# polli-labs/linnaeus

Hardware: AMD Instinct MI355X
Metric: images/sec (train fwd+bwd) mFormerV1_sm 3x224x224 (higher is better)
Workload: dtype bf16; 1 GPU; mFormerV1_sm train step (forward + 4-task CE loss + backward + AdamW (one HIP launch)), bf16 operands / fp32 accumulate+residual, batch 256/GPU, 3x224x224 synthetic, DropPath 0.2, gradient checkpointing off; per_gpu_batch=256, global_batch=256, parallelism=dp1, grad_mode=direct

## Files before the change

### include/lnx.h

```cpp
#ifndef LNX_H
#define LNX_H
#include <stdint.h>

#ifdef __cplusplus
extern "C" {
#endif

#define LNX_F32 0
#define LNX_BF16 1

const char* lnx_last_error(void);
int lnx_version(void);
int lnx_device_cus(void);
int lnx_set_cu_margin(int cus);
int lnx_set_deterministic(int on);
int lnx_get_deterministic(void);
int lnx_tile_sched_static(void);

typedef struct lnx_rowmap {
    int group, pad, off;
} lnx_rowmap;

enum { LNX_ACT_NONE = 0, LNX_ACT_GELU = 1, LNX_ACT_RELU = 2, LNX_ACT_GELU_BWD = 3, LNX_ACT_RELU_BWD = 4,
       LNX_ACT_GELU_D = 5, LNX_ACT_MUL_AUX = 6 };
// ... 898 lines not shown
    const float* mean;
    const float* rstd;
    float* d_ln_w;
    float* d_ln_b;
    float* ws;
    int64_t ws_floats;
    int dz_plain;
    int ln_defer;
    const int* perm;
    const int* m_dev;
} lnx_convmlp_bwd_args;
int lnx_convmlp_bwd(const lnx_convmlp_bwd_args* args, void* stream);
int64_t lnx_convmlp_bwd_ws_floats(int C, int M);


#define LNX_MAX_META 8
#define LNX_MAX_TASKS 16
typedef struct lnx_mformer_cfg {
    int dtype;
    int batch, img_h, img_w, in_chans;
    int dims[4];
    int conv_depths[2];
    int rope_depths[2];
    int rope_heads[2];
    int mlp_hidden[2];
    int n_meta;
    int meta_dims[LNX_MAX_META];
    int only_last_cls;
    int n_tasks;
    int task_classes[LNX_MAX_TASKS];
// ... 54 lines not shown
```

### linnaeus_amd/_lib.py

```python
from __future__ import annotations

import ctypes as C
import os

_HERE = os.path.dirname(os.path.abspath(__file__))
LIB_PATH = os.environ.get("LNX_LIB_PATH") or os.path.join(_HERE, "liblnx_hip.so")

F32, BF16 = 0, 1
ACT_NONE, ACT_GELU, ACT_RELU, ACT_GELU_BWD, ACT_RELU_BWD, ACT_GELU_D, ACT_MUL_AUX = 0, 1, 2, 3, 4, 5, 6
TN_WS_FLOATS = 256 * (256 * 128 + 256)
DROP_PARTITION_MAX = 64


def drop_list_ints(B: int) -> int:
    return 2 * B + 2
ADDR_PLAIN, ADDR_PATCH2 = 0, 1


class LnxError(RuntimeError):
    pass


class RowMap(C.Structure):
    _fields_ = [("group", C.c_int), ("pad", C.c_int), ("off", C.c_int)]
# ... 357 lines not shown
            _lib.lnx_plan_unit_name.argtypes = [C.c_void_p, C.c_int]
            _lib.lnx_plan_unit_name.restype = C.c_char_p
            _lib.lnx_plan_set_trainable.argtypes = [C.c_void_p, C.c_char_p]
        if hasattr(_lib, "lnx_plan_set_input_grads"):
            _lib.lnx_plan_set_input_grads.argtypes = [C.c_void_p, C.c_int, C.c_int]
            _lib.lnx_plan_input_grads.argtypes = [C.c_void_p]
            _lib.lnx_plan_bind_input_grads.argtypes = [C.c_void_p, C.c_void_p, C.c_void_p]
            _lib.lnx_stem_dgrad.argtypes = [C.POINTER(StemDgradArgs), C.c_void_p]
            _lib.lnx_col2im_stem.argtypes = [C.c_void_p, C.c_int, C.c_int, C.c_int, C.c_int, C.c_int, C.c_int, C.c_void_p, C.c_void_p]
            _lib.lnx_meta_input_grad.argtypes = [C.POINTER(MetaInputGradArgs), C.c_int, C.c_void_p, C.c_int, C.c_int, C.c_void_p]
        if hasattr(_lib, "lnx_gemm_tn_query"):
            _lib.lnx_gemm_tn_query.argtypes = [C.POINTER(WgradArgs), C.POINTER(TnLaunch)]
        if hasattr(_lib, "lnx_layernorm_fwd_query"):
            _lib.lnx_layernorm_fwd_query.argtypes = [C.POINTER(LnArgs), C.POINTER(LnLaunch)]
            _lib.lnx_layernorm_bwd_query.argtypes = [C.POINTER(LnBwdArgs), C.POINTER(LnLaunch)]
        older = bool(os.environ.get("LNX_LIB_PATH")) and os.environ.get("LNX_LIB_OLDER") == "1"
        for name in EXPORTS:
            if not hasattr(_lib, name) and not older:
                raise LnxError(f"{LIB_PATH} does not export {name}; rebuild it")
    return _lib


def set_deterministic(on: bool) -> bool:
    return bool(lib().lnx_set_deterministic(1 if on else 0))


def is_deterministic() -> bool:
    return bool(lib().lnx_get_deterministic())


# ... 11 lines not shown
ATTN_KERNEL_NONE, ATTN_KERNEL_RES4, ATTN_KERNEL_RES8, ATTN_KERNEL_TILED4, ATTN_KERNEL_TILED8 = range(5)

EXPORTS = [
    "lnx_last_error", "lnx_version", "lnx_device_cus", "lnx_set_cu_margin", "lnx_set_deterministic", "lnx_get_deterministic", "lnx_tile_sched_static",
    "lnx_gemm_nt", "lnx_last_nt_kernel", "lnx_nt_kernel_launches", "lnx_nt_dispatch", "lnx_gemm_tn", "lnx_gemm_tn_query", "lnx_gemm_tn_flush", "lnx_gemm_tn_discard", "lnx_amax", "lnx_quantize_fp8", "lnx_gemm_nt_fp8", "lnx_quantize_mxfp8", "lnx_gemm_nt_mxfp8", "lnx_dropout_mul", "lnx_dropout_residual", "lnx_plan_dropout_bytes", "lnx_plan_set_dropout", "lnx_plan_attn_dropout_bytes", "lnx_plan_set_attn_dropout",
    "lnx_layernorm_fwd", "lnx_layernorm_bwd", "lnx_layernorm_bwd_flush", "lnx_layernorm_bwd_discard", "lnx_layernorm_fwd_query", "lnx_layernorm_bwd_query",
    "lnx_dwconv7_fwd", "lnx_dwconv7_fwd_kept", "lnx_dwconv7_wgrad", "lnx_dwconv7_wgrad_kept", "lnx_dwconv7_wgrad_ws_floats",
    "lnx_gemm_nt_group_ok", "lnx_gemm_nt_group", "lnx_rope_cos_table", "lnx_rope_cos_table_hd", "lnx_rope_cossin_table_hd", "lnx_rope_cos_tables", "lnx_attn_bwd_ws_floats", "lnx_attn_bwd_ws_floats_hd", "lnx_attn_fwd", "lnx_attn_bwd", "lnx_attn_bwd_sized", "lnx_attn_fwd_compact", "lnx_attn_bwd_compact", "lnx_attn_bwd_flush", "lnx_attn_bwd_discard", "lnx_attn_dispatch", "lnx_last_attn_kernel", "lnx_last_attn_bwd_launches",
    "lnx_im2col_stem", "lnx_scale_cast", "lnx_scale_cast_compact", "lnx_drop_partition", "lnx_copy_dropped_rows", "lnx_set_drop_compact", "lnx_drop_compact_branches", "lnx_drop_compact_conv_blocks", "lnx_set_last_cls", "lnx_last_cls_blocks", "lnx_layerscale_bwd", "lnx_layerscale_bwd_ws", "lnx_layerscale_bwd_ws_floats", "lnx_layerscale_apply_wgrad", "lnx_fill_rows", "lnx_colsum_rows",
    "lnx_agg2_fwd", "lnx_agg2_bwd", "lnx_pack_meta", "lnx_meta_heads_supported", "lnx_meta_heads_fwd", "lnx_meta_heads_bwd", "lnx_meta_heads_bwd_part_floats", "lnx_prep_weights", "lnx_prep_blocks", "lnx_softce", "lnx_softce_multi", "lnx_taxonomy_rows", "lnx_stem_fwd", "lnx_stem_fwd_ok", "lnx_adamw_blocks", "lnx_grad_sumsq", "lnx_adamw_step", "lnx_ademamix_step", "lnx_sgd_step", "lnx_optim_launches", "lnx_grad_sumsq_guarded", "lnx_adamw_step_guarded", "lnx_ademamix_step_guarded", "lnx_sgd_step_guarded", "lnx_muon_layout", "lnx_muon_step", "lnx_muon_launches", "lnx_muon_partition", "lnx_muon_orthogonalize", "lnx_muon_apply_packed", "lnx_gradnorm_sumsq", "lnx_gradnorm_update",
    "lnx_metrics_table_sizes", "lnx_metrics_update", "lnx_predict", "lnx_resize_taps", "lnx_resize_coeffs", "lnx_preprocess_scratch_bytes", "lnx_preprocess", "lnx_hier_loss_fwd", "lnx_hier_loss_bwd",
    "lnx_hier_refine_fwd", "lnx_hier_refine_bwd", "lnx_hier_refine_launches",
    "lnx_abstain_act", "lnx_ppo_advantages", "lnx_ppo_loss_fwd", "lnx_ppo_loss_bwd", "lnx_abstain_launches",
    "lnx_mix_rows", "lnx_mix_meta", "lnx_meta_mask",
    "lnx_aug_pointwise", "lnx_aug_saturation", "lnx_aug_rowstat", "lnx_aug_rescale", "lnx_aug_affine", "lnx_aug_stencil", "lnx_erase_rects", "lnx_u8hwc_to_f32chw",
    "lnx_convmlp_supported", "lnx_convmlp_fwd", "lnx_convmlp_bwd", "lnx_convmlp_bwd_ws_floats",
    "lnx_plan_create", "lnx_plan_destroy", "lnx_plan_workspace_bytes", "lnx_plan_num_params", "lnx_plan_param_name",
    "lnx_plan_param_numel", "lnx_plan_num_drop_calls", "lnx_plan_logits_numel", "lnx_plan_logits_offset", "lnx_plan_logits_ld",
    "lnx_plan_bind", "lnx_plan_forward", "lnx_plan_forward_tail", "lnx_plan_trunk_valid", "lnx_plan_backward", "lnx_plan_backward_into", "lnx_plan_segment_params", "lnx_plan_profile_begin", "lnx_plan_profile_end", "lnx_plan_profile_begin_spans", "lnx_plan_profile_end_ex", "lnx_plan_set_wgrad_stream", "lnx_plan_set_meta_stream",
    "lnx_plan_num_units", "lnx_plan_unit_name", "lnx_plan_param_unit", "lnx_plan_set_trainable", "lnx_plan_first_trained_unit", "lnx_plan_last_backward_units",
    "lnx_stem_dgrad_ok", "lnx_stem_dgrad", "lnx_col2im_stem", "lnx_meta_input_grad", "lnx_plan_set_input_grads", "lnx_plan_input_grads", "lnx_plan_bind_input_grads",
]


class MetaHeadArgs(C.Structure):
    _fields_ = [
        ("B", C.c_int), ("C", C.c_int), ("dim", C.c_int), ("off", C.c_int),
        ("meta", C.c_void_p), ("meta_width", C.c_int), ("eps", C.c_float),
        ("w0", C.c_void_p), ("ldw0", C.c_int), ("b0", C.c_void_p), ("ln0_w", C.c_void_p), ("ln0_b", C.c_void_p),
        ("w1", C.c_void_p), ("ldw1", C.c_int), ("b1", C.c_void_p), ("ln1_w", C.c_void_p), ("ln1_b", C.c_void_p),
        ("w2", C.c_void_p), ("ldw2", C.c_int), ("b2", C.c_void_p), ("ln2_w", C.c_void_p), ("ln2_b", C.c_void_p),
# ... 124 lines not shown


class ConvMlpBwdArgs(C.Structure):
    _fields_ = [
        ("dtype", C.c_int), ("M", C.c_int), ("C", C.c_int),
        ("g", C.c_void_p), ("ln", C.c_void_p), ("z", C.c_void_p), ("w1", C.c_void_p), ("b1", C.c_void_p),
        ("w2t", C.c_void_p), ("w1t", C.c_void_p), ("gamma", C.c_void_p), ("rowscale", C.c_void_p), ("rows_per_sample", C.c_int),
        ("act", C.c_void_p), ("dh", C.c_void_p), ("dz", C.c_void_p), ("dln", C.c_void_p), ("dgamma", C.c_void_p),
        ("y", C.c_void_p), ("ln_w", C.c_void_p), ("mean", C.c_void_p), ("rstd", C.c_void_p), ("d_ln_w", C.c_void_p), ("d_ln_b", C.c_void_p),
        ("ws", C.c_void_p), ("ws_floats", C.c_int64),
        ("dz_plain", C.c_int), ("ln_defer", C.c_int),
        ("perm", C.c_void_p), ("m_dev", C.c_void_p),
    ]


class StemArgs(C.Structure):
    _fields_ = [("x", C.c_void_p), ("w", C.c_void_p), ("bias", C.c_void_p), ("ln_w", C.c_void_p), ("ln_b", C.c_void_p), ("patches", C.c_void_p),
                ("pre", C.c_void_p), ("y", C.c_void_p), ("mean", C.c_void_p), ("rstd", C.c_void_p), ("B", C.c_int), ("Cin", C.c_int), ("H", C.c_int),
                ("W", C.c_int), ("Cout", C.c_int), ("eps", C.c_float)]


class StemDgradArgs(C.Structure):
    _fields_ = [("dtype", C.c_int), ("B", C.c_int), ("Cin", C.c_int), ("H", C.c_int), ("W", C.c_int), ("Cout", C.c_int),
                ("dy", C.c_void_p), ("ldy", C.c_int64), ("w", C.c_void_p), ("dx", C.c_void_p)]


class MetaInputGradArgs(C.Structure):
    _fields_ = [("B", C.c_int), ("C", C.c_int), ("dim", C.c_int), ("off", C.c_int), ("dp0", C.c_void_p), ("lddp0", C.c_int64), ("w0", C.c_void_p), ("ldw0", C.c_int)]


# ... 20 lines not shown
```

### linnaeus_amd/csrc/api.cpp

```cpp
#include <hip/hip_runtime.h>
#include <stdarg.h>
#include <stdio.h>
#include <stdlib.h>
#include <string.h>

#include <atomic>
#include <mutex>

#include "../../include/lnx.h"

static thread_local char g_err[1024] = "";

void lnx_set_error(const char* fmt, ...) {
    va_list ap;
    va_start(ap, fmt);
    vsnprintf(g_err, sizeof(g_err), fmt, ap);
    va_end(ap);
}

extern "C" const char* lnx_last_error(void) { return g_err; }
extern "C" int lnx_version(void) { return 121; }
extern "C" int lnx_device_cus(void) {
    int dev = 0;
    if (hipGetDevice(&dev) != hipSuccess) return -1;
    hipDeviceProp_t prop;
    if (hipGetDeviceProperties(&prop, dev) != hipSuccess) return -1;
    return prop.multiProcessorCount;
}

static std::atomic<int> g_cu_margin{-1};
int persistent_cus(int cus) {
    int m = g_cu_margin.load(std::memory_order_relaxed);
    if (m < 0) {
        const char* e = getenv("LNX_CU_MARGIN");
        m = e ? atoi(e) : 0;
        if (m < 0) m = 0;
// ... 60 lines not shown
```

### linnaeus_amd/csrc/common.hpp

```cpp
#pragma once
#include <hip/hip_runtime.h>
#include <stdint.h>
#include <stdio.h>

typedef __bf16 bf16_t;
typedef __attribute__((ext_vector_type(8))) __bf16 bf16x8_t;
typedef __attribute__((ext_vector_type(4))) float f32x4_t;

#define LNX_WAVE 64

void lnx_set_error(const char* fmt, ...);

#define LNX_CHECK(cond, ...)                 \
    do {                                     \
        if (!(cond)) {                       \
            lnx_set_error(__VA_ARGS__);      \
            return 1;                        \
        }                                    \
    } while (0)

#define LNX_HIP(expr)                                                                  \
    do {                                                                               \
        hipError_t e_ = (expr);                                                        \
        if (e_ != hipSuccess) {                                                        \
// ... 220 lines not shown
#pragma unroll
    for (int i = 0; i < N; ++i) {
        const f32x2_t u = v[i] * splat2(K);
        const f32x2_t nuu = -(u * u);
        ex[i].x = __builtin_amdgcn_exp2f(nuu.x);
        ex[i].y = __builtin_amdgcn_exp2f(nuu.y);
    }
    erf_sqrt2_poly2_n<N>(v, e);
#pragma unroll
    for (int i = 0; i < N; ++i) {
        const f32x2_t cdf = e[i] * splat2(0.5f) + splat2(0.5f);
        act[i] = v[i] * cdf;
        dgelu[i] = (v[i] * splat2(0.39894228040143267794f)) * ex[i] + cdf;
    }
}
template <int K>
__device__ __forceinline__ void gelu4_bias_n(f32x4_t* h, const f32x4_t* b) {
    f32x2_t v[2 * K], a[2 * K];
#pragma unroll
    for (int k = 0; k < K; ++k) {
        v[2 * k] = f32x2_t{h[k][0] + b[k][0], h[k][1] + b[k][1]};
        v[2 * k + 1] = f32x2_t{h[k][2] + b[k][2], h[k][3] + b[k][3]};
    }
    gelu_lean2_n<2 * K>(v, a);
#pragma unroll
    for (int k = 0; k < K; ++k) h[k] = f32x4_t{a[2 * k].x, a[2 * k].y, a[2 * k + 1].x, a[2 * k + 1].y};
}
template <int K>
__device__ __forceinline__ void gelu4_bias_grad_n(f32x4_t* h, const f32x4_t* b, f32x4_t* da) {
    f32x2_t v[2 * K], a[2 * K], d[2 * K];
// ... 117 lines not shown
```

### linnaeus_amd/csrc/convmlp.hip

```cpp
#include <stdlib.h>

#include "common.hpp"
#include "../../include/lnx.h"

namespace {

struct CmP {
    const unsigned char* ln;
    const unsigned char* w1;
    const unsigned char* w2;
    const unsigned char* w2t;
    const unsigned char* w1t;
    const unsigned char* zin;
    const float* b1;
    const float* b2;
    const float* gamma;
    const float* rowscale;
    const float* x;
    const float* g;
    float* out;
    unsigned char* z;
    unsigned char* act;
    unsigned char* dh;
    unsigned char* dz;
// ... 941 lines not shown
                const float z0 = o[ct][mt][0] + b2.x, z1 = o[ct][mt][1] + b2.y, z2 = o[ct][mt][2] + b2.z, z3 = o[ct][mt][3] + b2.w;
                if constexpr (SAVE == 1) {
                    uint2 zz;
                    bf16_t* zh = reinterpret_cast<bf16_t*>(&zz);
                    zh[0] = (bf16_t)z0; zh[1] = (bf16_t)z1; zh[2] = (bf16_t)z2; zh[3] = (bf16_t)z3;
                    *reinterpret_cast<uint2*>(p.z + ((int64_t)m * C + c) * 2) = zz;
                }
                *reinterpret_cast<float4*>(p.out + (int64_t)m * C + c) =
                    make_float4(xr.x + rs * gm.x * z0, xr.y + rs * gm.y * z1, xr.z + rs * gm.z * z2, xr.w + rs * gm.w * z3);
            }
        }
    }
    if (reset_ctr && lane == 0) sched_reset(ctr);
}

template <int NK, int MT, bool ST, bool LNB, bool DG>
__global__ __launch_bounds__(512) void convmlp_bwd_res_kernel(const CmP p) {
    constexpr int C = Geo<NK>::C;
    constexpr int CT = Geo<NK>::CT;
    constexpr int PART = Geo<NK>::PART;
    constexpr int NCH = 4 * C / 64;
    extern __shared__ __attribute__((aligned(16))) unsigned char smem[];
    unsigned char* w1img = smem;
    unsigned char* w2timg = smem + NCH * PART;
    float* b1s = reinterpret_cast<float*>(smem + 2 * NCH * PART);
    float* dgs = b1s + 4 * C;
    float* lws = dgs + C;
    float* dls = lws + C;
    float* gms = dls + 2 * C;
    const int lane = threadIdx.x & 63;
    const int wave = __builtin_amdgcn_readfirstlane(threadIdx.x >> 6);
// ... 122 lines not shown
                for (int n2 = 0; n2 < 4; n2 += 2) {
                    f32x4_t hv[2] = {h[n2][mt], h[n2 + 1][mt]}, dv[2] = {da[n2][mt], da[n2 + 1][mt]};
                    gelu4_bias_grad_n<2>(hv, &bv[n2], dv);
                    h[n2][mt] = hv[0];
                    h[n2 + 1][mt] = hv[1];
                    da[n2][mt] = dv[0];
                    da[n2 + 1][mt] = dv[1];
                }
            uint4 pd[MT][2];
#pragma unroll
            for (int mt = 0; mt < MT; ++mt) {
                const uint4 pa0 = pack8(h[0][mt], h[1][mt]), pa1 = pack8(h[2][mt], h[3][mt]);
                pd[mt][0] = pack8(da[0][mt], da[1][mt]);
                pd[mt][1] = pack8(da[2][mt], da[3][mt]);
                const int m = min(m_base + mt * 16 + s, Me - 1);
                if constexpr (ST) {
                    const int64_t off = ((int64_t)m * (4 * C) + 64 * j + 8 * g) * 2;
                    st16(p.act + off, pa0);
                    st16(p.act + off + 64, pa1);
                    st16(p.dh + off, pd[mt][0]);
                    st16(p.dh + off + 64, pd[mt][1]);
                }
            }
            prod_tr_nmajor<NK, MT>(dl, lds0 + j * PART, s, g, pd);
        }
        __builtin_amdgcn_sched_barrier(0);
        if (dyn) {
            next = __builtin_amdgcn_readfirstlane(drawn);
            reset_ctr = reset_ctr || next == last_draw;
        } else {
            next = pos + xwaves;
        }
        fetch_tile(cur, next < xcnt ? xbase + next : tile);
        if constexpr (LNB) {
// ... 116 lines not shown
    if (p.y) return p.z ? launch_fwd_res_t<NK, true, 1>(p, st) : (p.ln_out ? launch_fwd_res_t<NK, true, 2>(p, st) : launch_fwd_res_t<NK, true, 0>(p, st));
    return p.z ? launch_fwd_res_t<NK, false, 1>(p, st) : launch_fwd_res_t<NK, false, 0>(p, st);
}
inline int reduce_ln_partials(const CmP& p, int nwg, hipStream_t st) {
    if (deterministic()) {
        ln_fold_rows(p.part, nwg, p.C, p.dlnw, p.dlnb, st);
        return 0;
    }
    if (p.ln_defer) {
        ln_postpone_reduce(p.part, nwg, p.C, p.dlnw, p.dlnb, nwg >= 64 ? 64 : 1, st);
        return 0;
    }
    hipLaunchKernelGGL(ln_partials_reduce_kernel, dim3(cdiv(2 * p.C, 256), nwg >= 64 ? 64 : 1), dim3(256), 0, st, p.part, nwg, p.C, p.dlnw, p.dlnb);
    return 0;
}
template <int NK, int MT, bool ST, bool LNB, bool DG>
int launch_bwd_res_t(const CmP& p, hipStream_t st) {
    const size_t lds0 = 2 * (4 * Geo<NK>::C / 64) * Geo<NK>::PART + 9 * Geo<NK>::C * sizeof(float);
    const size_t lds_det = lds0 + (LNB ? 8 * 2 * Geo<NK>::C * sizeof(float) : 0);
    static bool attr = false;
    if (!attr) {
        (void)hipFuncSetAttribute(reinterpret_cast<const void*>(&convmlp_bwd_res_kernel<NK, MT, ST, LNB, DG>), hipFuncAttributeMaxDynamicSharedMemorySize, (int)lds_det);
        attr = true;
    }
    int grid = bwd_grid(p.C, p.M);
    CmP q = p;
    if (bwd_scratch<LNB, DG>(q, grid) != 0) return -1;
    const int room = res_room();
    if (grid > room) grid = room;
    q.tile_slot = tile_sched_static() ? -1 : tile_slot_of(st);
    hipLaunchKernelGGL((convmlp_bwd_res_kernel<NK, MT, ST, LNB, DG>), dim3(grid), dim3(512), q.det ? lds_det : lds0, st, q);
    fold_dgamma(q, grid, st);
    return LNB ? reduce_ln_partials(p, q.det ? grid * 8 : grid, st) : 0;
}
template <int NK, int MT>
int launch_bwd_res(const CmP& p, hipStream_t st) {
    if (p.zin == nullptr) {
        if (p.y) return p.act ? launch_bwd_res_t<NK, MT, true, true, false>(p, st) : launch_bwd_res_t<NK, MT, false, true, false>(p, st);
        return p.act ? launch_bwd_res_t<NK, MT, true, false, false>(p, st) : launch_bwd_res_t<NK, MT, false, false, false>(p, st);
    }
    if (p.y) return p.act ? launch_bwd_res_t<NK, MT, true, true, true>(p, st) : launch_bwd_res_t<NK, MT, false, true, true>(p, st);
    return p.act ? launch_bwd_res_t<NK, MT, true, false, true>(p, st) : launch_bwd_res_t<NK, MT, false, false, true>(p, st);
}

template <int NK, int MT, int NW, bool LNF>
int launch_fwd_t(const CmP& p, hipStream_t st) {
    const size_t lds = 3 * 2 * Geo<NK>::PART + 4 * Geo<NK>::C * sizeof(float);
    static bool attr = false;
    if (!attr) {
        (void)hipFuncSetAttribute(reinterpret_cast<const void*>(&convmlp_fwd_kernel<NK, MT, NW, LNF>), hipFuncAttributeMaxDynamicSharedMemorySize, (int)lds);
        attr = true;
    }
    hipLaunchKernelGGL((convmlp_fwd_kernel<NK, MT, NW, LNF>), dim3(cdiv(p.M, 16 * NW * MT)), dim3(64 * NW), lds, st, p);
    return 0;
}
template <int NK, int MT, int NW>
int launch_fwd(const CmP& p, hipStream_t st) {
// ... 57 lines not shown
    hipStream_t st = (hipStream_t)stream;
    switch (a->C) {
        case 32: launch_fwd_res<1>(p, st); break;
        case 64: launch_fwd_res<2>(p, st); break;
        case 96: launch_fwd_res<3>(p, st); break;
        case 128: if (nw8) launch_fwd<4, 1, 8>(p, st); else launch_fwd<4, 1, 4>(p, st); break;
        case 192: if (nw8) launch_fwd<6, 1, 8>(p, st); else launch_fwd<6, 1, 4>(p, st); break;
    }
    LNX_LAUNCH_CHECK();
    return 0;
}

extern "C" int lnx_convmlp_bwd(const lnx_convmlp_bwd_args* a, void* stream) {
    LNX_CHECK(a && a->g && a->ln && a->w1 && a->w2t && a->w1t && a->b1 && a->gamma && a->dz && a->dln && (a->dgamma || !a->z),
              "lnx_convmlp_bwd: null operand (z may be NULL: dgamma is then not produced here; with z, dgamma is required)");
    LNX_CHECK((a->act == nullptr) == (a->dh == nullptr), "lnx_convmlp_bwd: act and dh must both be given or both be NULL");
    LNX_CHECK(lnx_convmlp_supported(a->dtype, a->C), "lnx_convmlp_bwd: unsupported dtype %d / C %d", a->dtype, a->C);
    LNX_CHECK(a->M > 0, "lnx_convmlp_bwd: empty");
    if (a->rowscale) LNX_CHECK(a->rows_per_sample > 0, "lnx_convmlp_bwd: rowscale needs rows_per_sample");
    if (a->z && deterministic()) LNX_CHECK(a->ws, "lnx_convmlp_bwd: deterministic mode needs ws (lnx_convmlp_bwd_ws_floats) for the waves' dgamma partial sums");
    if (a->y) LNX_CHECK(a->ln_w && a->mean && a->rstd && a->d_ln_w && a->d_ln_b && a->ws, "lnx_convmlp_bwd: the fused LayerNorm form needs ln_w, mean, rstd, d_ln_w, d_ln_b and ws");
    CmP p{};
    p.y = (const unsigned char*)a->y; p.lnw = a->ln_w; p.mean = const_cast<float*>(a->mean); p.rstd = const_cast<float*>(a->rstd);
    p.part = a->ws; p.part_floats = a->ws_floats; p.dlnw = a->d_ln_w; p.dlnb = a->d_ln_b; p.ln_defer = a->ln_defer;
    p.g = a->g; p.ln = (const unsigned char*)a->ln; p.zin = (const unsigned char*)a->z; p.w1 = (const unsigned char*)a->w1;
    p.w2t = (const unsigned char*)a->w2t; p.w1t = (const unsigned char*)a->w1t; p.b1 = a->b1; p.gamma = a->gamma; p.rowscale = a->rowscale;
    p.act = (unsigned char*)a->act; p.dh = (unsigned char*)a->dh; p.dz = (unsigned char*)a->dz; p.dln = (unsigned char*)a->dln; p.dgamma = a->dgamma;
    p.M = a->M; p.C = a->C; p.rps = a->rows_per_sample > 0 ? a->rows_per_sample : 1;
    p.dz_plain = a->dz_plain != 0;
    LNX_CHECK((a->perm == nullptr) == (a->m_dev == nullptr), "lnx_convmlp_bwd: perm and m_dev go together");
    if (a->perm) LNX_CHECK(a->rows_per_sample > 0 && a->M % a->rows_per_sample == 0 && a->z == nullptr, "lnx_convmlp_bwd: compact rows need rows_per_sample | M and no z");
    p.perm = a->perm; p.m_dev = a->m_dev;
// ... 14 lines not shown
```

### linnaeus_amd/csrc/plan.cpp

```cpp
#include <hip/hip_runtime.h>
#include <stdlib.h>
#include <string.h>

#include <mutex>
#include <atomic>
#include <string>
#include <vector>

#include "../../include/lnx.h"

void lnx_set_error(const char* fmt, ...);

#define RUN(expr)                  \
    do {                           \
        const int rc_ = (expr);    \
        if (rc_ != 0) return rc_;  \
    } while (0)
#define FAIL(...)                   \
    do {                            \
        lnx_set_error(__VA_ARGS__); \
        return 1;                   \
    } while (0)
#define HIPRUN(expr)                                                         \
    do {                                                                     \
// ... 1888 lines not shown
    const int M = B * H * W;
    void* sA = c.at<void>(p->o_sA);
    void* sC = c.at<void>(p->o_sC);
    void* sD = c.at<void>(p->o_sD);
    Timed span(c, 9, 4.0 * M * C * (8.0 * C + 49.0));
    bool forked = false, joined = false;
    const Compact cl = conv_compact_of(p, s, i);
    if (k.fused) {
        void* sB = c.at<void>(p->o_sB);
        lnx_convmlp_bwd_args f;
        memset(&f, 0, sizeof f);
        f.dtype = c.dt; f.M = M; f.C = C;
        f.g = g; f.ln = c.at<void>(k.ln); f.w1 = c.wptr(k.w1); f.b1 = p->P[k.b1];
        f.w2t = c.wtptr(k.w2); f.w1t = c.wtptr(k.w1); f.gamma = p->P[k.gamma];
        f.rowscale = p->drop_ptr(p->drop_conv[s][i]); f.rows_per_sample = H * W;
        f.act = sB; f.dh = sA; f.dz = sC; f.dln = sD; f.dgamma = p->G[k.gamma];
        f.dz_plain = 1;
        f.perm = cl.perm; f.m_dev = cl.m_dev;
        if (k.fused_ln) {
            f.y = c.at<void>(k.y); f.ln_w = p->P[k.lnw]; f.mean = c.at<float>(k.mean); f.rstd = c.at<float>(k.rstd);
            f.d_ln_w = p->G[k.lnw]; f.d_ln_b = p->G[k.lnb];
            f.ws = c.at<float>(p->o_lnws); f.ws_floats = p->lnws_floats;
            if (p->ln_defer && p->o_lnws_defer != 0 && lnx_convmlp_bwd_ws_floats(C, M) <= p->lnws_defer_floats) {
                RUN(ln_defer_slot(c, f.ws, f.ws_floats));
                f.ln_defer = 1;
            }
        }
        {
            Timed t(c, 7, 2.0 * M * C * 4 * C * 3);
            RUN(lnx_convmlp_bwd(&f, c.st));
        }
        const Ctx cw = wg_ctx(c);
        RUN(wg_fork(c, 0));
        forked = true;
        float* S = c.at<float>(p->o_lsws);
        float* T = S + (int64_t)C * 4 * C;
        HIPRUN(hipMemsetAsync(S, 0, ((size_t)C * 4 * C + C) * 4, (hipStream_t)cw.st));
        RUN(wgrad_into(cw, M, C, 4 * C, sC, C, sB, 4 * C, S, T, 4 * C, 0, cl.m_dev));
        RUN(wgrad(cw, M, 4 * C, C, sA, 4 * C, c.at<void>(k.ln), C, k.w1.param, k.b1, C, 0, 1, cl.m_dev));
        RUN(lnx_gemm_tn_flush(cw.st));
        RUN(lnx_layerscale_apply_wgrad(S, T, 4 * C, p->P[k.w2.param], p->P[k.b2], 4 * C, p->P[k.gamma], p->G[k.w2.param], p->G[k.b2], 4 * C, p->G[k.gamma], C, 4 * C, cw.st));
        RUN(wg_done(c, 0));
        if (!k.fused_ln) {
            RUN(wg_join(c, 0));
            joined = true;
        }
    } else {
        RUN(lnx_layerscale_bwd_ws(g, c.at<void>(k.z), c.dt, p->P[k.gamma], p->drop_ptr(p->drop_conv[s][i]), H * W, sC, p->G[k.gamma], M, C,
                                  p->det ? c.at<float>(p->o_detws) : nullptr, p->detws_floats, c.st));
        RUN(wgrad(c, M, C, 4 * C, sC, C, c.at<void>(k.act), 4 * C, k.w2.param, k.b2, 4 * C));
        lnx_gemm_args a = gemm_base(c, M, 4 * C, C, sC, C, c.wtptr(k.w2), k.w2.ld_t, sA, 4 * C, false);
        a.act = LNX_ACT_MUL_AUX; a.aux = c.at<void>(k.hpre); a.ldaux = 4 * C;
        RUN(gemm_nt_t(c, &a));
// ... 444 lines not shown
```

### linnaeus_amd/ops.py

```python
from __future__ import annotations

import ctypes as C
from typing import Optional, Tuple

import torch

from . import _lib as L
from ._lib import F32, BF16

_TORCH_DT = {F32: torch.float32, BF16: torch.bfloat16}


def code_of(t: torch.Tensor) -> int:
    if t.dtype == torch.float32:
        return F32
    if t.dtype == torch.bfloat16:
        return BF16
    raise L.LnxError(f"unsupported tensor dtype {t.dtype}")


def torch_dtype(code: int) -> torch.dtype:
    return _TORCH_DT[code]


# ... 485 lines not shown
                                               C.c_int64(dw.stride(0)), _p(dgamma), w.shape[0], w.shape[1], _stream()), "lnx_layerscale_apply_wgrad")


def convmlp_bwd(g, ln, z, w1, b1, w2t, w1t, gamma, act, dh, dz, dln, dgamma, *, rowscale=None, rows_per_sample=0, y=None, ln_w=None, mean=None,
                rstd=None, d_ln_w=None, d_ln_b=None, ws=None, dz_plain=False, ln_defer=False, perm=None, m_dev=None):
    a = L.ConvMlpBwdArgs()
    a.dtype, a.M, a.C = code_of(ln), ln.shape[0], ln.shape[1]
    a.g, a.ln, a.z, a.w1, a.b1, a.w2t, a.w1t, a.gamma = _p(g), _p(ln), _p(z), _p(w1), _p(b1), _p(w2t), _p(w1t), _p(gamma)
    a.rowscale, a.rows_per_sample = _p(rowscale), rows_per_sample
    a.act, a.dh, a.dz, a.dln, a.dgamma = _p(act), _p(dh), _p(dz), _p(dln), _p(dgamma)
    a.y, a.ln_w, a.mean, a.rstd, a.d_ln_w, a.d_ln_b = _p(y), _p(ln_w), _p(mean), _p(rstd), _p(d_ln_w), _p(d_ln_b)
    a.ws, a.ws_floats = _p(ws), (ws.numel() if ws is not None else 0)
    a.dz_plain, a.ln_defer = int(dz_plain), int(ln_defer)
    a.perm, a.m_dev = _p(perm), _p(m_dev)
    L.check(L.lib().lnx_convmlp_bwd(C.byref(a), _stream()), "lnx_convmlp_bwd")


def _meta_head_buffers(B, C_, dev):
    f = lambda *shape: torch.empty(*shape, device=dev, dtype=torch.float32)
    return {"t0": f(B, 16), "h0": f(B, C_), "x": f(B, C_), "h1": f(B, C_), "n1": f(B, C_), "h2": f(B, C_),
            "m0": f(B), "r0": f(B), "m1": f(B), "r1": f(B), "m2": f(B), "r2": f(B)}


def meta_heads_fwd(meta, heads, tok, eps=1e-5):
    B = meta.shape[0]
    arr = (L.MetaHeadArgs * len(heads))()
    keep, saved = [], []
    for i, h in enumerate(heads):
        C_ = h["w1"].shape[0]
        w0p = torch.zeros(C_, 16, device=meta.device)
# ... 210 lines not shown
```

Before: 14070 images/sec.

## Recompute GELU activation inside conv-MLP fc2 wgrad instead of storing act

For conv blocks with C <= 96 (bf16, non-deterministic), the backward kernel no longer writes the GELU activation tensor. A new persistent wgrad kernel recomputes h = GELU(ln·W1 + b1) on the fly with weights held in registers and accumulates dz^T·act and column sums via MFMA, finishing with float atomics. This trades the write and reread of the large M×4C activation for extra GEMM and GELU compute on the side wgrad stream. It is on by default unless disabled through an env var, and its float-atomic reduction makes results order-dependent.

```diff
diff --git a/include/lnx.h b/include/lnx.h
--- a/include/lnx.h
+++ b/include/lnx.h
@@ -936,6 +936,19 @@
 int64_t lnx_convmlp_bwd_ws_floats(int C, int M);
 
 
+typedef struct lnx_convmlp_wgrad2_args {
+    int dtype, M, C;
+    const void* ln;
+    const void* dz;
+    const void* w1;
+    const float* b1;
+    float* s;
+    float* t;
+    const int* m_dev;
+} lnx_convmlp_wgrad2_args;
+int lnx_convmlp_wgrad2(const lnx_convmlp_wgrad2_args* args, void* stream);
+int64_t lnx_convmlp_wgrad2_launches(void);
+
 #define LNX_MAX_META 8
 #define LNX_MAX_TASKS 16
 typedef struct lnx_mformer_cfg {
diff --git a/linnaeus_amd/_lib.py b/linnaeus_amd/_lib.py
--- a/linnaeus_amd/_lib.py
+++ b/linnaeus_amd/_lib.py
@@ -395,6 +395,9 @@
         if hasattr(_lib, "lnx_layernorm_fwd_query"):
             _lib.lnx_layernorm_fwd_query.argtypes = [C.POINTER(LnArgs), C.POINTER(LnLaunch)]
             _lib.lnx_layernorm_bwd_query.argtypes = [C.POINTER(LnBwdArgs), C.POINTER(LnLaunch)]
+        if hasattr(_lib, "lnx_convmlp_wgrad2"):
+            _lib.lnx_convmlp_wgrad2.argtypes = [C.POINTER(ConvMlpWgrad2Args), C.c_void_p]
+            _lib.lnx_convmlp_wgrad2_launches.restype = C.c_int64
         older = bool(os.environ.get("LNX_LIB_PATH")) and os.environ.get("LNX_LIB_OLDER") == "1"
         for name in EXPORTS:
             if not hasattr(_lib, name) and not older:
@@ -436,7 +439,7 @@
     "lnx_abstain_act", "lnx_ppo_advantages", "lnx_ppo_loss_fwd", "lnx_ppo_loss_bwd", "lnx_abstain_launches",
     "lnx_mix_rows", "lnx_mix_meta", "lnx_meta_mask",
     "lnx_aug_pointwise", "lnx_aug_saturation", "lnx_aug_rowstat", "lnx_aug_rescale", "lnx_aug_affine", "lnx_aug_stencil", "lnx_erase_rects", "lnx_u8hwc_to_f32chw",
-    "lnx_convmlp_supported", "lnx_convmlp_fwd", "lnx_convmlp_bwd", "lnx_convmlp_bwd_ws_floats",
+    "lnx_convmlp_supported", "lnx_convmlp_fwd", "lnx_convmlp_bwd", "lnx_convmlp_bwd_ws_floats", "lnx_convmlp_wgrad2", "lnx_convmlp_wgrad2_launches",
     "lnx_plan_create", "lnx_plan_destroy", "lnx_plan_workspace_bytes", "lnx_plan_num_params", "lnx_plan_param_name",
     "lnx_plan_param_numel", "lnx_plan_num_drop_calls", "lnx_plan_logits_numel", "lnx_plan_logits_offset", "lnx_plan_logits_ld",
     "lnx_plan_bind", "lnx_plan_forward", "lnx_plan_forward_tail", "lnx_plan_trunk_valid", "lnx_plan_backward", "lnx_plan_backward_into", "lnx_plan_segment_params", "lnx_plan_profile_begin", "lnx_plan_profile_end", "lnx_plan_profile_begin_spans", "lnx_plan_profile_end_ex", "lnx_plan_set_wgrad_stream", "lnx_plan_set_meta_stream",
@@ -591,6 +594,14 @@
     ]
 
 
+class ConvMlpWgrad2Args(C.Structure):
+    _fields_ = [
+        ("dtype", C.c_int), ("M", C.c_int), ("C", C.c_int),
+        ("ln", C.c_void_p), ("dz", C.c_void_p), ("w1", C.c_void_p), ("b1", C.c_void_p),
+        ("s", C.c_void_p), ("t", C.c_void_p), ("m_dev", C.c_void_p),
+    ]
+
+
 class StemArgs(C.Structure):
     _fields_ = [("x", C.c_void_p), ("w", C.c_void_p), ("bias", C.c_void_p), ("ln_w", C.c_void_p), ("ln_b", C.c_void_p), ("patches", C.c_void_p),
                 ("pre", C.c_void_p), ("y", C.c_void_p), ("mean", C.c_void_p), ("rstd", C.c_void_p), ("B", C.c_int), ("Cin", C.c_int), ("H", C.c_int),
diff --git a/linnaeus_amd/csrc/api.cpp b/linnaeus_amd/csrc/api.cpp
--- a/linnaeus_amd/csrc/api.cpp
+++ b/linnaeus_amd/csrc/api.cpp
@@ -19,7 +19,7 @@
 }
 
 extern "C" const char* lnx_last_error(void) { return g_err; }
-extern "C" int lnx_version(void) { return 121; }
+extern "C" int lnx_version(void) { return 122; }
 extern "C" int lnx_device_cus(void) {
     int dev = 0;
     if (hipGetDevice(&dev) != hipSuccess) return -1;
diff --git a/linnaeus_amd/csrc/common.hpp b/linnaeus_amd/csrc/common.hpp
--- a/linnaeus_amd/csrc/common.hpp
+++ b/linnaeus_amd/csrc/common.hpp
@@ -258,6 +258,16 @@
         dgelu[i] = (v[i] * splat2(0.39894228040143267794f)) * ex[i] + cdf;
     }
 }
+template <int N>
+__device__ __forceinline__ void gelu_lean_act2_n(const f32x2_t (&v)[N], f32x2_t (&act)[N]) {
+    f32x2_t e[N];
+    erf_sqrt2_poly2_n<N>(v, e);
+#pragma unroll
+    for (int i = 0; i < N; ++i) {
+        const f32x2_t cdf = e[i] * splat2(0.5f) + splat2(0.5f);
+        act[i] = v[i] * cdf;
+    }
+}
 template <int K>
 __device__ __forceinline__ void gelu4_bias_n(f32x4_t* h, const f32x4_t* b) {
     f32x2_t v[2 * K], a[2 * K];
diff --git a/linnaeus_amd/csrc/convmlp.hip b/linnaeus_amd/csrc/convmlp.hip
--- a/linnaeus_amd/csrc/convmlp.hip
+++ b/linnaeus_amd/csrc/convmlp.hip
@@ -979,7 +979,7 @@
     if (reset_ctr && lane == 0) sched_reset(ctr);
 }
 
-template <int NK, int MT, bool ST, bool LNB, bool DG>
+template <int NK, int MT, int ST, bool LNB, bool DG>
 __global__ __launch_bounds__(512) void convmlp_bwd_res_kernel(const CmP p) {
     constexpr int C = Geo<NK>::C;
     constexpr int CT = Geo<NK>::CT;
@@ -1132,10 +1132,12 @@
                 pd[mt][0] = pack8(da[0][mt], da[1][mt]);
                 pd[mt][1] = pack8(da[2][mt], da[3][mt]);
                 const int m = min(m_base + mt * 16 + s, Me - 1);
-                if constexpr (ST) {
+                if constexpr (ST != 0) {
                     const int64_t off = ((int64_t)m * (4 * C) + 64 * j + 8 * g) * 2;
-                    st16(p.act + off, pa0);
-                    st16(p.act + off + 64, pa1);
+                    if constexpr (ST == 1) {
+                        st16(p.act + off, pa0);
+                        st16(p.act + off + 64, pa1);
+                    }
                     st16(p.dh + off, pd[mt][0]);
                     st16(p.dh + off + 64, pd[mt][1]);
                 }
@@ -1282,7 +1284,7 @@
     hipLaunchKernelGGL(ln_partials_reduce_kernel, dim3(cdiv(2 * p.C, 256), nwg >= 64 ? 64 : 1), dim3(256), 0, st, p.part, nwg, p.C, p.dlnw, p.dlnb);
     return 0;
 }
-template <int NK, int MT, bool ST, bool LNB, bool DG>
+template <int NK, int MT, int ST, bool LNB, bool DG>
 int launch_bwd_res_t(const CmP& p, hipStream_t st) {
     const size_t lds0 = 2 * (4 * Geo<NK>::C / 64) * Geo<NK>::PART + 9 * Geo<NK>::C * sizeof(float);
     const size_t lds_det = lds0 + (LNB ? 8 * 2 * Geo<NK>::C * sizeof(float) : 0);
@@ -1304,11 +1306,11 @@
 template <int NK, int MT>
 int launch_bwd_res(const CmP& p, hipStream_t st) {
     if (p.zin == nullptr) {
-        if (p.y) return p.act ? launch_bwd_res_t<NK, MT, true, true, false>(p, st) : launch_bwd_res_t<NK, MT, false, true, false>(p, st);
-        return p.act ? launch_bwd_res_t<NK, MT, true, false, false>(p, st) : launch_bwd_res_t<NK, MT, false, false, false>(p, st);
-    }
-    if (p.y) return p.act ? launch_bwd_res_t<NK, MT, true, true, true>(p, st) : launch_bwd_res_t<NK, MT, false, true, true>(p, st);
-    return p.act ? launch_bwd_res_t<NK, MT, true, false, true>(p, st) : launch_bwd_res_t<NK, MT, false, false, true>(p, st);
+        if (p.y) return p.act ? launch_bwd_res_t<NK, MT, 1, true, false>(p, st) : (p.dh ? launch_bwd_res_t<NK, MT, 2, true, false>(p, st) : launch_bwd_res_t<NK, MT, 0, true, false>(p, st));
+        return p.act ? launch_bwd_res_t<NK, MT, 1, false, false>(p, st) : (p.dh ? launch_bwd_res_t<NK, MT, 2, false, false>(p, st) : launch_bwd_res_t<NK, MT, 0, false, false>(p, st));
+    }
+    if (p.y) return p.act ? launch_bwd_res_t<NK, MT, 1, true, true>(p, st) : (p.dh ? launch_bwd_res_t<NK, MT, 2, true, true>(p, st) : launch_bwd_res_t<NK, MT, 0, true, true>(p, st));
+    return p.act ? launch_bwd_res_t<NK, MT, 1, false, true>(p, st) : (p.dh ? launch_bwd_res_t<NK, MT, 2, false, true>(p, st) : launch_bwd_res_t<NK, MT, 0, false, true>(p, st));
 }
 
 template <int NK, int MT, int NW, bool LNF>
@@ -1396,8 +1398,10 @@
 extern "C" int lnx_convmlp_bwd(const lnx_convmlp_bwd_args* a, void* stream) {
     LNX_CHECK(a && a->g && a->ln && a->w1 && a->w2t && a->w1t && a->b1 && a->gamma && a->dz && a->dln && (a->dgamma || !a->z),
               "lnx_convmlp_bwd: null operand (z may be NULL: dgamma is then not produced here; with z, dgamma is required)");
-    LNX_CHECK((a->act == nullptr) == (a->dh == nullptr), "lnx_convmlp_bwd: act and dh must both be given or both be NULL");
+    LNX_CHECK(a->act == nullptr || a->dh != nullptr, "lnx_convmlp_bwd: act without dh is not a form the kernels are built for (both, neither, or dh alone at C <= 96)");
     LNX_CHECK(lnx_convmlp_supported(a->dtype, a->C), "lnx_convmlp_bwd: unsupported dtype %d / C %d", a->dtype, a->C);
+    LNX_CHECK(a->act != nullptr || a->dh == nullptr || a->C <= 96,
+              "lnx_convmlp_bwd: dh without act is built for the weight-resident kernels only (C <= 96, here C = %d): act and dh must both be given or both be NULL", a->C);
     LNX_CHECK(a->M > 0, "lnx_convmlp_bwd: empty");
     if (a->rowscale) LNX_CHECK(a->rows_per_sample > 0, "lnx_convmlp_bwd: rowscale needs rows_per_sample");
     if (a->z && deterministic()) LNX_CHECK(a->ws, "lnx_convmlp_bwd: deterministic mode needs ws (lnx_convmlp_bwd_ws_floats) for the waves' dgamma partial sums");
diff --git a/linnaeus_amd/csrc/convmlp_wgrad2.hip b/linnaeus_amd/csrc/convmlp_wgrad2.hip
--- /dev/null
+++ b/linnaeus_amd/csrc/convmlp_wgrad2.hip
@@ -0,0 +1,217 @@
+#include <stdlib.h>
+
+#include <atomic>
+
+#include "common.hpp"
+#include "../../include/lnx.h"
+
+namespace {
+
+struct W2P {
+    const unsigned char* ln;
+    const unsigned char* dz;
+    const unsigned char* w1;
+    const float* b1;
+    float* s;
+    float* t;
+    const int* m_dev;
+    int M;
+};
+
+__device__ const uint4 g_w2_zero16 = {0u, 0u, 0u, 0u};
+
+__device__ __forceinline__ int key4(int a) { return (4 - (a & 3)) & 3; }
+
+__device__ __forceinline__ void mfma16(f32x4_t& acc, const uint4& a, const uint4& b) {
+    acc = __builtin_amdgcn_mfma_f32_16x16x32_bf16(__builtin_bit_cast(bf16x8_t, a), __builtin_bit_cast(bf16x8_t, b), acc, 0, 0, 0);
+}
+__device__ __forceinline__ uint4 pack8(const f32x4_t& lo, const f32x4_t& hi) {
+    Vec16<bf16_t> v;
+#pragma unroll
+    for (int j = 0; j < 4; ++j) {
+        v.set(j, lo[j]);
+        v.set(4 + j, hi[j]);
+    }
+    return v.raw;
+}
+
+constexpr int W2_ROWS = 64;
+constexpr int W2_NST = 3;
+
+template <int NK>
+__global__ __launch_bounds__(512) void convmlp_wgrad2_kernel(const W2P p) {
+    constexpr int C = 32 * NK;
+    constexpr int NT = NK;
+    constexpr int CT = 2 * NK;
+    constexpr int IMG = NK * 4096;
+    constexpr int STG = 2 * IMG;
+    extern __shared__ __attribute__((aligned(16))) unsigned char smem[];
+    const int lane = threadIdx.x & 63;
+    const int wave = __builtin_amdgcn_readfirstlane(threadIdx.x >> 6);
+    const int s = lane & 15, g = lane >> 4;
+    const uint32_t lds0 = (uint32_t)(uintptr_t)(__attribute__((address_space(3))) unsigned char*)smem;
+
+    const int Me = p.m_dev ? min(max(__builtin_amdgcn_readfirstlane(*p.m_dev), 0), p.M) : p.M;
+    const int total = (Me + W2_ROWS - 1) / W2_ROWS;
+    const int first = (int)blockIdx.x, grid = (int)gridDim.x;
+    const int nst = first < total ? (total - first + grid - 1) / grid : 0;
+    if (nst == 0) return;
+
+    auto issue = [&](int t) __attribute__((always_inline)) {
+        const int64_t m0 = ((int64_t)first + (int64_t)t * grid) * W2_ROWS;
+        unsigned char* dst = smem + (t % W2_NST) * STG;
+#pragma unroll
+        for (int j = 0; j < NK; ++j) {
+            const int i = wave + 8 * j;
+            const int r = i % (4 * NK);
+            const int ks = r >> 2, rb = r & 3;
+            const int row = 16 * rb + (lane >> 2), u = lane & 3;
+            const int64_t m = m0 + row;
+            const unsigned char* src = (i >= 4 * NK ? p.dz : p.ln) + (m * C + ks * 32 + ((u ^ key4(row >> 2)) << 3)) * 2;
+            if (t >= nst || m >= Me) src = reinterpret_cast<const unsigned char*>(&g_w2_zero16);
+            __builtin_amdgcn_global_load_lds((const __attribute__((address_space(1))) void*)src, (__attribute__((address_space(3))) void*)(dst + i * 1024), 16, 0, 0);
+        }
+    };
+    issue(0);
+    issue(1);
+
+    const int nb = wave * (C / 2);
+    uint4 wf[NT][NK];
+    float bv[NT];
+#pragma unroll
+    for (int nt = 0; nt < NT; ++nt) {
+#pragma unroll
+        for (int ks = 0; ks < NK; ++ks) wf[nt][ks] = ld16(p.w1 + ((int64_t)(nb + 16 * nt + s) * C + ks * 32 + 8 * g) * 2);
+        bv[nt] = p.b1[nb + 16 * nt + s];
+    }
+    f32x4_t S[CT][NT];
+#pragma unroll
+    for (int ct = 0; ct < CT; ++ct)
+#pragma unroll
+        for (int nt = 0; nt < NT; ++nt) S[ct][nt] = f32x4_t{0.f, 0.f, 0.f, 0.f};
+    f32x4_t tacc = f32x4_t{0.f, 0.f, 0.f, 0.f};
+    const uint4 ones = make_uint4(0x3F803F80u, 0x3F803F80u, 0x3F803F80u, 0x3F803F80u);
+
+    const int q = s >> 2, pp = s & 3;
+    const uint32_t xoff = (uint32_t)(s * 64 + ((g ^ key4(s >> 2)) << 4));
+    uint32_t zoff[2];
+#pragma unroll
+    for (int e = 0; e < 2; ++e) zoff[e] = (uint32_t)(IMG + (4 * g + q) * 64 + (((2 * e + (pp >> 1)) ^ key4(g)) << 4) + (pp & 1) * 8);
+
+    for (int t = 0; t < nst; ++t) {
+        asm volatile("s_waitcnt vmcnt(%0)" ::"n"(NK) : "memory");
+        __builtin_amdgcn_s_barrier();
+        __builtin_amdgcn_sched_barrier(0);
+        issue(t + 2);
+        const uint32_t st = lds0 + (uint32_t)((t % W2_NST) * STG);
+#pragma unroll
+        for (int half = 0; half < 2; ++half) {
+            const uint32_t r0 = st + (uint32_t)(half * 32 * 64);
+            uint4 xf[2][NK];
+#pragma unroll
+            for (int mt = 0; mt < 2; ++mt)
+#pragma unroll
+                for (int ks = 0; ks < NK; ++ks) {
+                    const uint32_t a = r0 + xoff + (uint32_t)(ks * 4096 + mt * 1024);
+                    asm volatile("ds_read_b128 %0, %1" : "=v"(xf[mt][ks]) : "v"(a) : "memory");
+                }
+            asm volatile("s_waitcnt lgkmcnt(0)" ::: "memory");
+            __builtin_amdgcn_sched_barrier(0);
+            f32x4_t h[2][NT];
+#pragma unroll
+            for (int mt = 0; mt < 2; ++mt)
+#pragma unroll
+                for (int nt = 0; nt < NT; ++nt) h[mt][nt] = f32x4_t{0.f, 0.f, 0.f, 0.f};
+#pragma unroll
+            for (int ks = 0; ks < NK; ++ks)
+#pragma unroll
+                for (int mt = 0; mt < 2; ++mt)
+#pragma unroll
+                    for (int nt = 0; nt < NT; ++nt) mfma16(h[mt][nt], xf[mt][ks], wf[nt][ks]);
+            uint2 lo[CT], hi[CT];
+#pragma unroll
+            for (int ct = 0; ct < CT; ++ct) {
+                const uint32_t a = r0 + zoff[ct & 1] + (uint32_t)((ct >> 1) * 4096);
+                asm volatile("ds_read_b64_tr_b16 %0, %1" : "=v"(lo[ct]) : "v"(a) : "memory");
+                asm volatile("ds_read_b64_tr_b16 %0, %1 offset:1024" : "=v"(hi[ct]) : "v"(a) : "memory");
+            }
+#pragma unroll
+            for (int mt = 0; mt < 2; ++mt) {
+                f32x2_t v[2 * NT], a[2 * NT];
+#pragma unroll
+                for (int nt = 0; nt < NT; ++nt) {
+                    v[2 * nt] = f32x2_t{h[mt][nt][0] + bv[nt], h[mt][nt][1] + bv[nt]};
+                    v[2 * nt + 1] = f32x2_t{h[mt][nt][2] + bv[nt], h[mt][nt][3] + bv[nt]};
+                }
+                gelu_lean_act2_n<2 * NT>(v, a);
+#pragma unroll
+                for (int nt = 0; nt < NT; ++nt) h[mt][nt] = f32x4_t{a[2 * nt].x, a[2 * nt].y, a[2 * nt + 1].x, a[2 * nt + 1].y};
+            }
+            uint4 pf[NT];
+#pragma unroll
+            for (int nt = 0; nt < NT; ++nt) pf[nt] = pack8(h[0][nt], h[1][nt]);
+            asm volatile("s_waitcnt lgkmcnt(0)" ::: "memory");
+            __builtin_amdgcn_sched_barrier(0);
+#pragma unroll
+            for (int ct = 0; ct < CT; ++ct) {
+                const uint4 af = make_uint4(lo[ct].x, lo[ct].y, hi[ct].x, hi[ct].y);
+#pragma unroll
+                for (int nt = 0; nt < NT; ++nt) mfma16(S[ct][nt], af, pf[nt]);
+                if (wave == ct) mfma16(tacc, af, ones);
+            }
+        }
+    }
+    asm volatile("s_waitcnt vmcnt(0)" ::: "memory");
+#pragma unroll
+    for (int ct = 0; ct < CT; ++ct) {
+#pragma unroll
+        for (int nt = 0; nt < NT; ++nt)
+#pragma unroll
+            for (int r = 0; r < 4; ++r) atomicAdd(p.s + (int64_t)(16 * ct + 4 * g + r) * (4 * C) + nb + 16 * nt + s, S[ct][nt][r]);
+    }
+    if (wave < CT && s == 0) {
+#pragma unroll
+        for (int r = 0; r < 4; ++r) atomicAdd(p.t + 16 * wave + 4 * g + r, tacc[r]);
+    }
+}
+
+std::atomic<long long> g_w2_launches{0};
+
+int w2_grid(int M) {
+    const int cus = device_cus();
+    int room = persistent_cus(cus > 0 ? cus : 256);
+    if (room > 256) room = 256;
+    const int steps = cdiv(M, W2_ROWS);
+    return steps < room ? steps : room;
+}
+
+template <int NK>
+int launch_w2(const W2P& p, hipStream_t st) {
+    return launch_with_lds<convmlp_wgrad2_kernel<NK>>(w2_grid(p.M), 512, (size_t)W2_NST * 2 * NK * 4096, st, p);
+}
+
+}
+
+extern "C" int64_t lnx_convmlp_wgrad2_launches(void) { return (int64_t)g_w2_launches.load(std::memory_order_relaxed); }
+
+extern "C" int lnx_convmlp_wgrad2(const lnx_convmlp_wgrad2_args* a, void* stream) {
+    LNX_CHECK(a && a->ln && a->dz && a->w1 && a->b1 && a->s && a->t, "lnx_convmlp_wgrad2: null operand (ln, dz, w1, b1, s and t are required)");
+    LNX_CHECK(a->dtype == LNX_BF16, "lnx_convmlp_wgrad2: bf16 only (dtype %d)", a->dtype);
+    LNX_CHECK(a->C == 32 || a->C == 64 || a->C == 96, "lnx_convmlp_wgrad2: unsupported C %d (the weight-resident conv blocks: C in {32, 64, 96})", a->C);
+    LNX_CHECK(a->M > 0, "lnx_convmlp_wgrad2: empty");
+    LNX_CHECK(!deterministic(), "lnx_convmlp_wgrad2: deterministic mode has no fixed-order route here (s and t are summed by float atomics): store act and use lnx_gemm_tn");
+    W2P p{};
+    p.ln = (const unsigned char*)a->ln; p.dz = (const unsigned char*)a->dz; p.w1 = (const unsigned char*)a->w1; p.b1 = a->b1;
+    p.s = a->s; p.t = a->t; p.m_dev = a->m_dev; p.M = a->M;
+    hipStream_t st = (hipStream_t)stream;
+    int rc = 0;
+    switch (a->C) {
+        case 32: rc = launch_w2<1>(p, st); break;
+        case 64: rc = launch_w2<2>(p, st); break;
+        case 96: rc = launch_w2<3>(p, st); break;
+    }
+    if (rc != 0) return rc;
+    LNX_LAUNCH_CHECK();
+    g_w2_launches.fetch_add(1, std::memory_order_relaxed);
+    return 0;
+}
diff --git a/linnaeus_amd/csrc/plan.cpp b/linnaeus_amd/csrc/plan.cpp
--- a/linnaeus_amd/csrc/plan.cpp
+++ b/linnaeus_amd/csrc/plan.cpp
@@ -1926,7 +1926,9 @@
         f.g = g; f.ln = c.at<void>(k.ln); f.w1 = c.wptr(k.w1); f.b1 = p->P[k.b1];
         f.w2t = c.wtptr(k.w2); f.w1t = c.wtptr(k.w1); f.gamma = p->P[k.gamma];
         f.rowscale = p->drop_ptr(p->drop_conv[s][i]); f.rows_per_sample = H * W;
-        f.act = sB; f.dh = sA; f.dz = sC; f.dln = sD; f.dgamma = p->G[k.gamma];
+        static const bool conv_noact = env_off("LNX_CONV_ACT");
+        const bool no_act = C <= 96 && c.dt == LNX_BF16 && !p->det && conv_noact;
+        f.act = no_act ? nullptr : sB; f.dh = sA; f.dz = sC; f.dln = sD; f.dgamma = p->G[k.gamma];
         f.dz_plain = 1;
         f.perm = cl.perm; f.m_dev = cl.m_dev;
         if (k.fused_ln) {
@@ -1948,7 +1950,16 @@
         float* S = c.at<float>(p->o_lsws);
         float* T = S + (int64_t)C * 4 * C;
         HIPRUN(hipMemsetAsync(S, 0, ((size_t)C * 4 * C + C) * 4, (hipStream_t)cw.st));
-        RUN(wgrad_into(cw, M, C, 4 * C, sC, C, sB, 4 * C, S, T, 4 * C, 0, cl.m_dev));
+        if (no_act) {
+            lnx_convmlp_wgrad2_args w2;
+            memset(&w2, 0, sizeof w2);
+            w2.dtype = c.dt; w2.M = M; w2.C = C;
+            w2.ln = f.ln; w2.dz = sC; w2.w1 = f.w1; w2.b1 = f.b1; w2.s = S; w2.t = T; w2.m_dev = cl.m_dev;
+            Timed t(cw, M >= 1024 ? 1 : -1, 2.0 * M * C * 4 * C, (double)p->esz * ((double)M * C + (double)M * 4 * C) + 8.0 * C * 4 * C);
+            RUN(lnx_convmlp_wgrad2(&w2, cw.st));
+        } else {
+            RUN(wgrad_into(cw, M, C, 4 * C, sC, C, sB, 4 * C, S, T, 4 * C, 0, cl.m_dev));
+        }
         RUN(wgrad(cw, M, 4 * C, C, sA, 4 * C, c.at<void>(k.ln), C, k.w1.param, k.b1, C, 0, 1, cl.m_dev));
         RUN(lnx_gemm_tn_flush(cw.st));
         RUN(lnx_layerscale_apply_wgrad(S, T, 4 * C, p->P[k.w2.param], p->P[k.b2], 4 * C, p->P[k.gamma], p->G[k.w2.param], p->G[k.b2], 4 * C, p->G[k.gamma], C, 4 * C, cw.st));
diff --git a/linnaeus_amd/ops.py b/linnaeus_amd/ops.py
--- a/linnaeus_amd/ops.py
+++ b/linnaeus_amd/ops.py
@@ -523,6 +523,15 @@
     a.dz_plain, a.ln_defer = int(dz_plain), int(ln_defer)
     a.perm, a.m_dev = _p(perm), _p(m_dev)
     L.check(L.lib().lnx_convmlp_bwd(C.byref(a), _stream()), "lnx_convmlp_bwd")
+
+
+def convmlp_wgrad2(ln, dz, w1, b1, s, t, *, m_dev=None, dtype=None, M=None, C_=None):
+    a = L.ConvMlpWgrad2Args()
+    a.dtype = dtype if dtype is not None else code_of(ln)
+    a.M, a.C = (M if M is not None else ln.shape[0]), (C_ if C_ is not None else ln.shape[1])
+    a.ln, a.dz, a.w1, a.b1, a.s, a.t, a.m_dev = _p(ln), _p(dz), _p(w1), _p(b1), _p(s), _p(t), _p(m_dev)
+    L.check(L.lib().lnx_convmlp_wgrad2(C.byref(a), _stream()), "lnx_convmlp_wgrad2")
+    return s, t
 
 
 def _meta_head_buffers(B, C_, dev):
```

Result: no change. 14000 images/sec (-0.5%).
